# jiangzhengkai/mxdetection

Measured on AMD Instinct MI355X. Metric: images/sec (whole node) Faster R-CNN R50-FPN 3x800x1333, higher is better.
Workload: dtype bf16; 1 GPU; Faster R-CNN ResNet-50-FPN bf16 train step, batch 2/GPU, 3x800x1333 (padded 1344); global_batch=2, parallelism=dp1, frozen=stem+C2, frozen BN folded, optimizer=SGD momentum 0.9 wd 1e-4, launch=hipGraph replay, input=resident, wgrad_side_stream=True, rpn_branch_stream=True, grouped_wgrad=True, filter_prefetch_hints=True, params_trainable=41538304

## Files before the change

include/mxdet.h:

```cpp
#ifndef MXDET_H_
#define MXDET_H_

#include <stddef.h>
#include <stdint.h>

#ifdef __cplusplus
extern "C" {
#endif

#define MXDET_OK 0
#define MXDET_EINVAL (-1)
#define MXDET_ESHAPE (-2)
#define MXDET_EWORKSPACE (-3)
#define MXDET_EHIP (-4)
#define MXDET_ERCCL (-5)

#define MXDET_DTYPE_F32 0
#define MXDET_DTYPE_BF16 1

typedef void* mxdet_stream_t;

const char* mxdet_last_error(void);
const char* mxdet_version(void);

// ... 205 lines not shown
                     const float* bias, const uint16_t* residual, uint16_t* y,
                     mxdet_stream_t stream);
int mxdet_conv2d_fwd_chain(const mxdet_conv_desc_t* d, const uint16_t* x, const uint16_t* w, const float* bias,
                           const uint16_t* w2, const float* bias2, int32_t cout2, int32_t relu2,
                           const uint16_t* residual2, uint16_t* y2, const uint16_t* w3, const float* bias3,
                           int32_t cout3, int32_t relu3, uint16_t* y3, mxdet_stream_t stream);
size_t mxdet_conv2d_fwd_splitk_workspace_bytes(const mxdet_conv_desc_t* d, int32_t ksplit);
int mxdet_conv2d_fwd_splitk(const mxdet_conv_desc_t* d, const uint16_t* x, const uint16_t* w, const float* bias,
                            const uint16_t* residual, uint16_t* y, int32_t ksplit, void* workspace,
                            size_t workspace_bytes, mxdet_stream_t stream);
int mxdet_conv2d_dgrad(const mxdet_conv_desc_t* d, const uint16_t* dy, const uint16_t* wt,
                       const uint16_t* residual, const uint16_t* relu_mask, uint16_t* dx,
                       mxdet_stream_t stream);
size_t mxdet_conv2d_wgrad_workspace_bytes(const mxdet_conv_desc_t* d);
int mxdet_conv2d_wgrad(const mxdet_conv_desc_t* d, const uint16_t* x, const uint16_t* dy, float* dw,
                       float* db, void* workspace, size_t workspace_bytes, mxdet_stream_t stream);
typedef struct {
  mxdet_conv_desc_t desc;
  const void* src;
  const void* filt;
  const float* bias;
  const void* residual;
  const void* relu_mask;
  void* dst;
} mxdet_conv_item_t;
size_t mxdet_conv2d_grouped_table_bytes(int32_t n);
int mxdet_conv2d_grouped_plan(const mxdet_conv_item_t* items, int32_t n, int32_t kind, void* table_host,
                              size_t table_bytes, int32_t* cfg, int32_t* grid);
int mxdet_conv2d_grouped(const void* table_dev, int32_t n, int32_t kind, int32_t cfg, int32_t grid,
                         mxdet_stream_t stream);
typedef struct {
  mxdet_conv_desc_t desc;
  const void* x;
  const void* dy;
  float* dw;
  float* db;
} mxdet_wgrad_item_t;
size_t mxdet_conv2d_wgrad_grouped_table_bytes(int32_t n);
int mxdet_conv2d_wgrad_grouped_plan(const mxdet_wgrad_item_t* items, int32_t n, void* table_host, size_t table_bytes,
                                    size_t* workspace_bytes, int32_t* grid_wgrad, int32_t* grid_big,
                                    int32_t* grid_reduce);
int mxdet_conv2d_wgrad_grouped(const void* table_dev, int32_t n, int32_t grid_wgrad, int32_t grid_big,
                               int32_t grid_reduce, void* workspace, size_t workspace_bytes, size_t workspace_needed,
                               mxdet_stream_t stream);
int mxdet_conv2d_wgrad_grouped_parts(const void* table_dev, int32_t n, int32_t grid_wgrad, int32_t grid_big,
                                     int32_t grid_reduce, int32_t parts, void* workspace, size_t workspace_bytes,
                                     size_t workspace_needed, mxdet_stream_t stream);
int mxdet_filter_transpose(const uint16_t* w, int32_t Cout, int32_t KH, int32_t KW, int32_t Cin,
                           uint16_t* wt, mxdet_stream_t stream);

int mxdet_filter_transpose_batched(const void* descs_dev, int32_t ndesc, int32_t total_tiles,
                                   mxdet_stream_t stream);

typedef struct {
  int32_t N, H, W, C;
  int32_t Ho, Wo;
  int32_t KH, KW;
  int32_t stride, pad;
  int32_t groups;
  int32_t modulated;
  int32_t off_channels;
  int32_t accumulate;
} mxdet_deform_desc_t;
int mxdet_deform_im2col(const mxdet_deform_desc_t* d, const uint16_t* x, const uint16_t* off, uint16_t* col,
                        mxdet_stream_t stream);
int mxdet_deform_col2im_coord(const mxdet_deform_desc_t* d, const uint16_t* x, const uint16_t* off,
                              const uint16_t* dcol, uint16_t* doff, mxdet_stream_t stream);
size_t mxdet_deform_col2im_workspace_bytes(const mxdet_deform_desc_t* d);
int mxdet_deform_col2im(const mxdet_deform_desc_t* d, const uint16_t* off, const uint16_t* dcol, uint16_t* dx,
                        void* workspace, size_t workspace_bytes, mxdet_stream_t stream);

typedef struct {
  int32_t N, HW, C, G;
  float eps;
  int32_t relu;
  int32_t accumulate;
} mxdet_gn_desc_t;
size_t mxdet_group_norm_workspace_bytes(const mxdet_gn_desc_t* d, int32_t backward);
int mxdet_group_norm_fwd(const mxdet_gn_desc_t* d, const uint16_t* x, const float* gamma, const float* beta, uint16_t* y,
                         float* mean, float* rstd, void* workspace, size_t workspace_bytes, mxdet_stream_t stream);
int mxdet_group_norm_bwd(const mxdet_gn_desc_t* d, const uint16_t* x, const uint16_t* dy, const uint16_t* y,
                         const float* mean, const float* rstd, const float* gamma, const float* beta, uint16_t* dx,
                         float* dgamma, float* dbeta, void* workspace, size_t workspace_bytes, mxdet_stream_t stream);

int mxdet_stem_conv7x7(const void* image, int32_t dtype, int32_t N, int32_t H, int32_t W,
                       const uint16_t* w, const float* bias, uint16_t* y, mxdet_stream_t stream);
int mxdet_stem_conv7x7_pool(const void* image, int32_t dtype, int32_t N, int32_t H, int32_t W,
                            const uint16_t* w, const float* bias, uint16_t* y, mxdet_stream_t stream);
int mxdet_maxpool3x3s2(const uint16_t* x, int32_t N, int32_t H, int32_t W, int32_t C, uint16_t* y,
                       mxdet_stream_t stream);
int mxdet_subsample2(const uint16_t* x, int32_t N, int32_t H, int32_t W, int32_t C, uint16_t* y,
                     mxdet_stream_t stream);
int mxdet_subsample2_bwd(const uint16_t* dy, int32_t N, int32_t H, int32_t W, int32_t C,
                         int32_t accumulate, uint16_t* dx, mxdet_stream_t stream);
int mxdet_upsample2_bwd(const uint16_t* dfine, int32_t N, int32_t Hf, int32_t Wf, int32_t C,
                        int32_t accumulate, uint16_t* dcoarse, mxdet_stream_t stream);
size_t mxdet_retina_detect_workspace_bytes(const mxdet_pyramid_t* p, int32_t N, int32_t pre_nms_top_n);
int mxdet_retina_detect(const mxdet_pyramid_t* p, int32_t N, const float* im_info, int32_t pre_nms_top_n,
                        float score_thresh, float nms_thresh, int32_t max_per_image, float* dets, int32_t* num_dets,
                        void* workspace, size_t workspace_bytes, mxdet_stream_t stream);
int mxdet_retina_detect_soft(const mxdet_pyramid_t* p, int32_t N, const float* im_info, int32_t pre_nms_top_n,
                             float score_thresh, float nms_thresh, int32_t max_per_image, float* dets,
                             int32_t* num_dets, void* workspace, size_t workspace_bytes, int32_t method, float sigma,
                             mxdet_stream_t stream);

typedef struct {
// ... 50 lines not shown
```

mxdetection_amd/_lib.py:

```python
import ctypes as C
import os

_HERE = os.path.dirname(os.path.abspath(__file__))
LIB_PATH = os.environ.get("MXDET_LIB") or os.path.join(_HERE, "libmxdet_hip.so")

c_i32, c_i64, c_u32, c_f32, c_sz, c_vp = C.c_int32, C.c_int64, C.c_uint32, C.c_float, C.c_size_t, C.c_void_p


class PyramidT(C.Structure):
    _fields_ = [
        ("num_levels", c_i32), ("A", c_i32),
        ("H", c_i32 * 8), ("W", c_i32 * 8), ("stride", c_i32 * 8),
        ("cls", c_vp * 8), ("reg", c_vp * 8),
        ("cls_sn", c_i64 * 8), ("cls_sy", c_i64 * 8), ("cls_sx", c_i64 * 8), ("cls_sa", c_i64 * 8),
        ("reg_sn", c_i64 * 8), ("reg_sy", c_i64 * 8), ("reg_sx", c_i64 * 8), ("reg_sc", c_i64 * 8),
        ("dtype", c_i32), ("classes", c_i32),
        ("base_anchors", c_vp * 8),
    ]


class FeatPyramidT(C.Structure):
    _fields_ = [
        ("num_levels", c_i32), ("lvl_min", c_i32),
        ("H", c_i32 * 8), ("W", c_i32 * 8),
        ("spatial_scale", c_f32 * 8),
        ("feat", c_vp * 8),
    ]


class ImageDescT(C.Structure):
    _fields_ = [("src", C.c_void_p), ("src_h", C.c_int32), ("src_w", C.c_int32), ("dst_h", C.c_int32),
                ("dst_w", C.c_int32), ("flip", C.c_int32), ("pad_", C.c_int32), ("inv_scale", C.c_double)]


class WgradItemT(C.Structure):
    pass


class ConvItemT(C.Structure):
    pass


class ConvDescT(C.Structure):
    _fields_ = [
        ("N", c_i32), ("H", c_i32), ("W", c_i32), ("Cin", c_i32),
        ("Cout", c_i32), ("KH", c_i32), ("KW", c_i32),
        ("stride", c_i32), ("pad", c_i32),
        ("Ho", c_i32), ("Wo", c_i32),
        ("relu", c_i32), ("res_upsample", c_i32), ("accumulate", c_i32),
        ("prefetch", c_vp), ("prefetch_bytes", c_i64), ("relu_bits", c_vp),
    ]


class DeformDescT(C.Structure):
    _fields_ = [
        ("N", c_i32), ("H", c_i32), ("W", c_i32), ("C", c_i32),
        ("Ho", c_i32), ("Wo", c_i32), ("KH", c_i32), ("KW", c_i32),
        ("stride", c_i32), ("pad", c_i32), ("groups", c_i32), ("modulated", c_i32),
        ("off_channels", c_i32), ("accumulate", c_i32),
    ]


class DpoolDescT(C.Structure):
    _fields_ = [
        ("pyr", FeatPyramidT), ("N", c_i32), ("C", c_i32), ("PH", c_i32), ("PW", c_i32),
        ("sample_per_part", c_i32), ("trans_std", c_f32), ("modulated", c_i32),
        ("trans_stride", c_i32), ("mask_stride", c_i32), ("accumulate", c_i32),
    ]


class GnDescT(C.Structure):
    _fields_ = [("N", c_i32), ("HW", c_i32), ("C", c_i32), ("G", c_i32), ("eps", c_f32), ("relu", c_i32),
                ("accumulate", c_i32)]


WgradItemT._fields_ = [("desc", ConvDescT), ("x", c_vp), ("dy", c_vp), ("dw", c_vp), ("db", c_vp)]
ConvItemT._fields_ = [("desc", ConvDescT), ("src", c_vp), ("filt", c_vp), ("bias", c_vp), ("residual", c_vp),
                      ("relu_mask", c_vp), ("dst", c_vp)]

P = C.POINTER

SIGNATURES = {
    "mxdet_last_error": (C.c_char_p, []),
    "mxdet_version": (C.c_char_p, []),
    "mxdet_box_iou": (c_i32, [c_vp, c_i64, c_vp, c_i64, c_vp, c_vp]),
    "mxdet_generate_anchors": (c_i32, [c_vp, c_i32, c_i32, c_i32, c_i32, c_vp, c_vp]),
    "mxdet_nms_batched_workspace_bytes": (c_sz, [c_i32, c_i32]),
    "mxdet_nms_batched": (c_i32, [c_vp, c_vp, c_vp, c_i32, c_i32, c_f32, c_i32, c_vp, c_vp, c_vp, c_sz, c_vp]),
    "mxdet_soft_nms_batched": (c_i32, [c_vp, c_vp, c_vp, c_i32, c_i32, c_i32, c_f32, c_f32, c_f32, c_i32, c_vp, c_vp, c_vp,
                                       c_vp]),
    "mxdet_pixel_shuffle2_inv_relu": (c_i32, [c_vp, c_vp, c_i64, c_i32, c_i32, c_i32, c_vp, c_vp]),
    "mxdet_mask_paste_workspace_bytes": (c_sz, [c_i64, c_i32]),
    "mxdet_mask_paste": (c_i32, [c_vp, c_vp, c_i64, c_i32, c_i32, c_i32, c_i32, c_f32, c_vp, c_vp, c_sz, c_vp]),
    "mxdet_retina_detect_workspace_bytes": (c_sz, [c_vp, c_i32, c_i32]),
    "mxdet_retina_detect": (c_i32, [c_vp, c_i32, c_vp, c_i32, c_f32, c_f32, c_i32, c_vp, c_vp, c_vp, c_sz, c_vp]),
    "mxdet_retina_detect_soft": (c_i32, [c_vp, c_i32, c_vp, c_i32, c_f32, c_f32, c_i32, c_vp, c_vp, c_vp, c_sz, c_i32, c_f32,
                                         c_vp]),
    "mxdet_debug_preprocess_direct": (c_i32, [c_i32]),
    "mxdet_image_preprocess": (c_i32, [c_vp, c_i32, c_i32, c_i32, c_vp, c_vp, c_i32, c_vp, c_vp]),
    "mxdet_polygon_masks": (c_i32, [c_vp, c_vp, c_vp, c_i32, c_i32, c_i32, c_i32, c_vp, c_vp]),
    "mxdet_detection_postprocess_workspace_bytes": (c_sz, [c_i32, c_i32, c_i32]),
    "mxdet_detection_postprocess": (c_i32, [c_vp, c_vp, c_i32, c_i32, c_i32, c_vp, c_vp, c_vp, c_i32, c_i32, c_i32,
                                            P(c_f32), P(c_f32), c_f32, c_f32, c_i32, c_vp, c_vp, c_vp, c_sz, c_vp]),
    "mxdet_detection_postprocess_soft": (c_i32, [c_vp, c_vp, c_i32, c_i32, c_i32, c_vp, c_vp, c_vp, c_i32, c_i32, c_i32,
                                                 P(c_f32), P(c_f32), c_f32, c_f32, c_i32, c_vp, c_vp, c_vp, c_sz, c_i32,
                                                 c_f32, c_vp]),
    "mxdet_proposal_workspace_bytes": (c_sz, [P(PyramidT), c_i32, c_i32]),
    "mxdet_proposal": (c_i32, [P(PyramidT), c_i32, c_vp, c_i32, c_i32, c_f32, c_f32, c_vp, c_vp, c_vp, c_vp,
                               c_vp, c_sz, c_vp]),
    "mxdet_anchor_target_workspace_bytes": (c_sz, [c_i32, c_i64, c_i32]),
    "mxdet_anchor_target": (c_i32, [c_vp, c_i64, c_vp, c_i32, c_i32, c_vp, c_f32, c_f32, c_f32, c_i32, c_f32,
                                    c_u32, c_u32, c_vp, c_u32, c_vp, c_vp, c_vp, c_vp, c_vp, c_sz, c_vp]),
    "mxdet_atss_assign_workspace_bytes": (c_sz, [c_i32, c_i64, c_i32]),
    "mxdet_atss_assign": (c_i32, [c_vp, c_i64, P(c_i64), c_i32, c_vp, c_i32, c_i32, c_i32, c_vp, c_vp, c_vp, c_vp, c_vp, c_sz,
                                  c_vp]),
    "mxdet_proposal_target": (c_i32, [c_vp, c_vp, c_i32, c_vp, c_i32, c_i32, c_i32, c_f32, c_f32, c_f32, c_f32,
                                      c_i32, c_i32, P(c_f32), P(c_f32), c_u32, c_u32, c_vp, c_u32, c_vp, c_vp, c_vp,
                                      c_vp, c_vp, c_vp, c_vp]),
    "mxdet_fpn_level_map": (c_i32, [c_vp, c_i64, c_i32, c_i32, c_vp, c_vp]),
    "mxdet_roi_align_fwd": (c_i32, [P(FeatPyramidT), c_i32, c_i32, c_vp, c_vp, c_i64, c_i32, c_i32, c_i32, c_vp,
                                    c_vp]),
    "mxdet_roi_align_bwd": (c_i32, [P(FeatPyramidT), c_i32, c_i32, c_vp, c_vp, c_i64, c_i32, c_i32, c_i32, c_vp,
                                    c_vp]),
    "mxdet_roi_align_bwd_gather_workspace_bytes": (c_sz, [P(FeatPyramidT), c_i32, c_i64]),
    "mxdet_roi_align_bwd_gather": (c_i32, [P(FeatPyramidT), c_i32, c_i32, c_vp, c_vp, c_i64, c_i32, c_i32, c_i32, c_vp,
                                           c_i32, c_vp, c_sz, c_vp]),
    "mxdet_roi_align_bwd_gather_prepare": (c_i32, [P(FeatPyramidT), c_i32, c_vp, c_vp, c_i64, c_i32, c_i32, c_i32,
                                                   c_vp, c_sz, c_vp]),
    "mxdet_roi_align_bwd_gather_prepared": (c_i32, [P(FeatPyramidT), c_i32, c_i32, c_vp, c_vp, c_i64, c_i32, c_i32, c_i32,
                                                    c_vp, c_i32, c_vp, c_sz, c_vp]),
    "mxdet_smooth_l1_fwd": (c_i32, [c_vp, c_vp, c_vp, c_i64, c_f32, c_vp, c_vp]),
    "mxdet_smooth_l1_bwd": (c_i32, [c_vp, c_vp, c_vp, c_vp, c_i64, c_f32, c_i32, c_vp, c_vp]),
    "mxdet_loss_workspace_bytes": (c_sz, [c_i64]),
    "mxdet_focal_loss": (c_i32, [c_vp, c_i32, c_vp, c_i64, c_i32, c_f32, c_f32, c_f32, c_vp, c_vp, c_vp, c_sz,
                                 c_vp]),
    "mxdet_anchor_class_labels": (c_i32, [c_vp, c_vp, c_vp, c_i32, c_i64, c_i32, c_vp, c_vp, c_vp]),
    "mxdet_retina_loss_num_partials": (c_i32, [c_i32, c_i32, c_i32, c_i32]),
    "mxdet_retina_loss_level": (c_i32, [c_vp, c_vp, c_i32, c_i32, c_i32, c_i32, c_i32, c_i32, c_i32, c_vp, c_vp, c_i64,
                                        c_i64, c_f32, c_f32, c_f32, c_vp, c_f32, c_vp, c_vp, c_vp, c_vp]),
    "mxdet_rpn_loss_num_partials": (c_i32, [c_i32, c_i32, c_i32]),
    "mxdet_rpn_loss_level": (c_i32, [c_vp, c_i32, c_i32, c_i32, c_i32, c_i32, c_vp, c_vp, c_i64, c_i64, c_f32,
                                     c_f32, c_f32, c_vp, c_vp, c_vp]),
    "mxdet_loss_finalize": (c_i32, [c_vp, c_i32, c_i32, c_vp, c_vp]),
    "mxdet_rcnn_loss": (c_i32, [c_vp, c_vp, c_i32, c_i32, c_i32, c_vp, c_vp, c_vp, c_i64, c_i32, c_i32, c_f32,
                                c_f32, c_f32, c_vp, c_vp, c_vp, c_vp, c_sz, c_vp]),
    "mxdet_box_iou_loss": (c_i32, [c_vp, c_vp, c_vp, c_i32, c_i32, c_vp, c_i64, c_i32, c_f32, c_f32, c_f32, c_f32, c_f32, c_vp,
                                   c_vp, c_vp]),
    "mxdet_rcnn_loss_iou": (c_i32, [c_vp, c_vp, c_i32, c_i32, c_i32, c_vp, c_vp, c_vp, c_vp, c_i32, c_i32, c_i64, c_i32, c_i32,
                                    c_i32, c_f32, c_f32, c_f32, c_f32, c_f32, c_f32, c_f32, c_vp, c_vp, c_vp, c_vp, c_sz,
                                    c_vp]),
    "mxdet_retina_loss_level_iou": (c_i32, [c_vp, c_vp, c_i32, c_i32, c_i32, c_i32, c_i32, c_i32, c_i32, c_vp, c_vp, c_vp, c_vp,
                                            c_i32, c_i64, c_i64, c_f32, c_f32, c_i32, c_f32, c_f32, c_f32, c_f32, c_f32, c_vp,
                                            c_f32, c_vp, c_vp, c_vp, c_vp]),
    "mxdet_mask_target": (c_i32, [c_vp, c_vp, c_vp, c_vp, c_i64, c_i32, c_i32, c_i32, c_i32, c_vp, c_vp, c_vp]),
    "mxdet_pixel_shuffle2": (c_i32, [c_vp, c_i64, c_i32, c_i32, c_i32, c_i32, c_vp, c_vp]),
    "mxdet_mask_loss_workspace_bytes": (c_sz, [c_i64, c_i32]),
    "mxdet_mask_loss": (c_i32, [c_vp, c_vp, c_vp, c_i64, c_i32, c_i32, c_f32, c_vp, c_vp, c_vp, c_sz, c_vp]),
    "mxdet_conv2d_fwd": (c_i32, [P(ConvDescT), c_vp, c_vp, c_vp, c_vp, c_vp, c_vp]),
    "mxdet_conv2d_fwd_chain": (c_i32, [P(ConvDescT), c_vp, c_vp, c_vp, c_vp, c_vp, c_i32, c_i32, c_vp, c_vp, c_vp, c_vp, c_i32,
                                       c_i32, c_vp, c_vp]),
    "mxdet_conv2d_fwd_splitk_workspace_bytes": (c_sz, [P(ConvDescT), c_i32]),
    "mxdet_conv2d_fwd_splitk": (c_i32, [P(ConvDescT), c_vp, c_vp, c_vp, c_vp, c_vp, c_i32, c_vp, c_sz, c_vp]),
    "mxdet_conv2d_dgrad": (c_i32, [P(ConvDescT), c_vp, c_vp, c_vp, c_vp, c_vp, c_vp]),
    "mxdet_conv2d_wgrad_workspace_bytes": (c_sz, [P(ConvDescT)]),
    "mxdet_conv2d_wgrad": (c_i32, [P(ConvDescT), c_vp, c_vp, c_vp, c_vp, c_vp, c_sz, c_vp]),
    "mxdet_conv2d_grouped_table_bytes": (c_sz, [c_i32]),
    "mxdet_conv2d_grouped_plan": (c_i32, [P(ConvItemT), c_i32, c_i32, c_vp, c_sz, P(c_i32), P(c_i32)]),
    "mxdet_conv2d_grouped": (c_i32, [c_vp, c_i32, c_i32, c_i32, c_i32, c_vp]),
    "mxdet_conv2d_wgrad_grouped_table_bytes": (c_sz, [c_i32]),
    "mxdet_conv2d_wgrad_grouped_plan": (c_i32, [P(WgradItemT), c_i32, c_vp, c_sz, P(c_sz), P(c_i32), P(c_i32), P(c_i32)]),
    "mxdet_conv2d_wgrad_grouped": (c_i32, [c_vp, c_i32, c_i32, c_i32, c_i32, c_vp, c_sz, c_sz, c_vp]),
    "mxdet_conv2d_wgrad_grouped_parts": (c_i32, [c_vp, c_i32, c_i32, c_i32, c_i32, c_i32, c_vp, c_sz, c_sz, c_vp]),
    "mxdet_debug_force_conv_cfg": (c_i32, [c_i32]),
    "mxdet_debug_force_wgrad_ksplit": (c_i32, [c_i32]),
    "mxdet_filter_transpose": (c_i32, [c_vp, c_i32, c_i32, c_i32, c_i32, c_vp, c_vp]),
    "mxdet_filter_transpose_batched": (c_i32, [c_vp, c_i32, c_i32, c_vp]),
    "mxdet_deform_im2col": (c_i32, [P(DeformDescT), c_vp, c_vp, c_vp, c_vp]),
    "mxdet_deform_col2im_coord": (c_i32, [P(DeformDescT), c_vp, c_vp, c_vp, c_vp, c_vp]),
    "mxdet_deform_col2im_workspace_bytes": (c_sz, [P(DeformDescT)]),
    "mxdet_deform_col2im": (c_i32, [P(DeformDescT), c_vp, c_vp, c_vp, c_vp, c_sz, c_vp]),
    "mxdet_dpool_fwd": (c_i32, [P(DpoolDescT), c_vp, c_vp, c_i64, c_vp, c_vp, c_vp, c_vp]),
    "mxdet_dpool_bwd_trans": (c_i32, [P(DpoolDescT), c_vp, c_vp, c_i64, c_vp, c_vp, c_vp, c_vp, c_vp, c_vp]),
    "mxdet_dpool_bwd_feat_workspace_bytes": (c_sz, [P(DpoolDescT), c_i64]),
    "mxdet_dpool_bwd_feat": (c_i32, [P(DpoolDescT), c_vp, c_vp, c_i64, c_vp, c_vp, c_vp, c_vp, c_sz, c_vp]),
    "mxdet_group_norm_workspace_bytes": (c_sz, [P(GnDescT), c_i32]),
    "mxdet_group_norm_fwd": (c_i32, [P(GnDescT), c_vp, c_vp, c_vp, c_vp, c_vp, c_vp, c_vp, c_sz, c_vp]),
    "mxdet_group_norm_bwd": (c_i32, [P(GnDescT), c_vp, c_vp, c_vp, c_vp, c_vp, c_vp, c_vp, c_vp, c_vp, c_vp, c_vp, c_sz,
                                     c_vp]),
    "mxdet_debug_group_norm_route": (c_i32, [P(GnDescT)]),
    "mxdet_stem_conv7x7": (c_i32, [c_vp, c_i32, c_i32, c_i32, c_i32, c_vp, c_vp, c_vp, c_vp]),
    "mxdet_stem_conv7x7_pool": (c_i32, [c_vp, c_i32, c_i32, c_i32, c_i32, c_vp, c_vp, c_vp, c_vp]),
    "mxdet_maxpool3x3s2": (c_i32, [c_vp, c_i32, c_i32, c_i32, c_i32, c_vp, c_vp]),
    "mxdet_subsample2": (c_i32, [c_vp, c_i32, c_i32, c_i32, c_i32, c_vp, c_vp]),
    "mxdet_subsample2_bwd": (c_i32, [c_vp, c_i32, c_i32, c_i32, c_i32, c_i32, c_vp, c_vp]),
    "mxdet_upsample2_bwd": (c_i32, [c_vp, c_i32, c_i32, c_i32, c_i32, c_i32, c_vp, c_vp]),
    "mxdet_add_bf16": (c_i32, [c_vp, c_vp, c_i64, c_vp, c_vp]),
    "mxdet_relu_bwd_bf16": (c_i32, [c_vp, c_vp, c_i64, c_vp, c_vp]),
    "mxdet_f32_to_bf16": (c_i32, [c_vp, c_i64, c_vp, c_vp]),
    "mxdet_f32_accum_to_bf16": (c_i32, [c_vp, c_i64, c_i32, c_vp, c_vp]),
    "mxdet_nchw_to_nhwc_bf16": (c_i32, [c_vp, c_i32, c_i32, c_i32, c_i32, c_i32, c_vp, c_vp]),
    "mxdet_nhwc_to_nchw_f32": (c_i32, [c_vp, c_i32, c_i32, c_i32, c_i32, c_vp, c_vp]),
    "mxdet_sgd_momentum_update": (c_i32, [c_vp, c_vp, c_vp, c_vp, c_i64, c_f32, c_f32, c_f32, c_f32, c_vp]),
    "mxdet_sgd_momentum_update_sched": (c_i32, [c_vp, c_vp, c_vp, c_vp, c_i64, c_vp, c_f32, c_f32, c_f32, c_vp]),
    "mxdet_comm_unique_id": (c_i32, [c_vp]),
    "mxdet_comm_create": (c_i32, [c_vp, c_i32, c_i32, P(c_vp)]),
    "mxdet_comm_destroy": (c_i32, [c_vp]),
    "mxdet_allreduce_bucket": (c_i32, [c_vp, c_vp, c_i64, c_vp, P(c_i32)]),
    "mxdet_comm_wait": (c_i32, [c_vp, c_i32, c_vp]),
    "mxdet_comm_broadcast": (c_i32, [c_vp, c_vp, c_sz, c_i32, c_vp]),
    "mxdet_debug_set_tuning": (c_i32, [c_i32, c_i64]),
    "mxdet_debug_get_tuning": (c_i64, [c_i32]),
    "mxdet_debug_route_probe": (c_i32, [c_i32]),
    "mxdet_debug_route_read": (c_i32, [P(c_i32), c_i32]),
}

DEBUG_SYMBOLS = ("mxdet_debug_force_conv_cfg", "mxdet_debug_force_wgrad_ksplit", "mxdet_debug_preprocess_direct",
                 "mxdet_debug_set_tuning", "mxdet_debug_get_tuning", "mxdet_debug_route_probe", "mxdet_debug_route_read",
                 "mxdet_debug_group_norm_route")
TUNING_KEYS = {"T64": 0, "T128": 1, "PAR64": 2, "WG_TARGET": 3, "WG_MINSTEPS": 4, "WG_MAXSTEPS": 5, "T3_ENABLE": 6,
               "T3_TARGET": 7, "T3_MINSTEPS": 8, "T3_NS": 9, "TAIL": 10, "WG_NS": 11, "ROI_TABLE": 12, "ROI_ROWS": 13, "STATIC_TAPS": 14,
               "T128W": 15, "T3_MIX": 16, "SPLITK_TILE": 17, "T3_PER_ITEM": 18}
ROUTE_KINDS = {"CONV": 1, "WGRAD": 2, "CONV_GROUPED": 3, "WGRAD_GROUPED": 4, "RETINA_LOSS": 5, "RETINA_LOSS_IOU": 6}

IOU_LOSS_KINDS = {"iou": 0, "giou": 1, "diou": 2}

_lib = None

# ... 43 lines not shown
```

mxdetection_amd/models/rpn_heads/rpn_head.py:

```python
import os

import torch

from ...core import anchor as A_
from ...core import loss as L_
from ...ops import dense
from ...ops.proposal import PyramidProposal
from ..utils.layers import ConvLayer, cached_buf

HEAD_CPAD = 64


RELU_BITS = os.environ.get("MXDET_TUNE_RELU_BITS", "1") == "1"


class RPNHead:
    def __init__(self, channels, strides, arena, ws, device, gen, ratios=(0.5, 1.0, 2.0), scales=(8,),
                 pre_nms_top_n=2000, post_nms_top_n=2000, nms_thresh=0.7, min_size=0.0, batch_size=256,
                 fg_fraction=0.5, fg_thresh=0.7, bg_thresh=0.3, sigma=3.0, seed=99):
        kw = dict(arena=arena, ws=ws, device=device, gen=gen)
        self.A = len(ratios) * len(scales)
        assert 5 * self.A <= HEAD_CPAD
        self.out = ConvLayer("rpn.out", channels, HEAD_CPAD, 1, init_std=0.01, cout_real=5 * self.A, **kw)
        self.conv = ConvLayer("rpn.conv", channels, channels, 3, init_std=0.01, **kw)
        self.strides = list(strides)
        self.base = [torch.from_numpy(A_.generate_base_anchors(s, ratios, scales)).to(device) for s in strides]
        self.proposal = PyramidProposal(self.base, strides, pre_nms_top_n, post_nms_top_n, nms_thresh, min_size)
        self.batch_size, self.fg_fraction, self.fg_thresh, self.bg_thresh = batch_size, fg_fraction, fg_thresh, bg_thresh
        self.sigma, self.seed, self.device, self.C = sigma, seed, device, channels
        self.bufs = {}
        self.anchors = None
        self.level_shapes = None

    def layers(self):
        return [self.out, self.conv]

    def _buf(self, key, shape, dtype=torch.bfloat16, zero=False):
        return cached_buf(self.bufs, key, shape, dtype, self.device, zero)

    def plan(self, p_shapes, g_max):
        for s in p_shapes:
            self.conv.plan(s)
            self.out.plan(s)
        self.level_shapes = [(s[1], s[2]) for s in p_shapes]
        N = p_shapes[0][0]
        self.anchors = torch.cat([A_.generate_anchors(self.base[l], H, W, self.strides[l])
                                  for l, (H, W) in enumerate(self.level_shapes)])
        self.level_offsets = [0]
        for (H, W) in self.level_shapes:
            self.level_offsets.append(self.level_offsets[-1] + H * W * self.A)
        At = self.anchors.shape[0]
        self.at_ws = A_.AnchorTargetWorkspace(N, At, g_max, self.device)
        self.at_out = (torch.empty((N, At), dtype=torch.int32, device=self.device),
                       torch.empty((N, At), dtype=torch.int32, device=self.device),
                       torch.empty((N, At, 4), dtype=torch.float32, device=self.device),
                       torch.empty((N, At), dtype=torch.float32, device=self.device))
        self.nparts = [L_.rpn_loss_num_partials(N, H, W) for (H, W) in self.level_shapes]
        self.partial = torch.zeros((2 * sum(self.nparts),), dtype=torch.float32, device=self.device)
        self.loss = torch.zeros((2,), dtype=torch.float32, device=self.device)

    def forward(self, P):
        self.P = P
        tb = [self._buf("t%d" % l, p.shape) for l, p in enumerate(P)]
        hb = [self._buf("h%d" % l, p.shape[:3] + (HEAD_CPAD,)) for l, p in enumerate(P)]
        self.tbits = [self._buf("tb%d" % l, p.shape[:3] + (p.shape[3] // 8,), dtype=torch.uint8) if RELU_BITS else None
                      for l, p in enumerate(P)]
        self.conv.forward(P[0], relu=True, out=tb[0], bits_out=self.tbits[0])
        dense.conv2d_group("fwd", [self.conv.fwd_call(P[l], relu=True, out=tb[l], bits_out=self.tbits[l])
                                   for l in range(1, len(P))], self.device)
        self.out.forward(tb[0], out=hb[0])
        dense.conv2d_group("fwd", [self.out.fwd_call(tb[l], out=hb[l]) for l in range(1, len(P))], self.device)
        self.t, self.h = tb, hb
        return self.h

    def get_proposals(self, im_info):
        return self.proposal(self.h, self.h, im_info, layout="nhwc_fused")

    def assign_targets(self, gt_boxes, im_info, step, image_offset, step_dev=None):
        labels, _, targets, _ = A_.assign_anchor(self.anchors, gt_boxes, im_info, self.fg_thresh, self.bg_thresh, 0.0,
                                                 self.batch_size, self.fg_fraction, self.seed, step, image_offset,
                                                 self.at_ws, self.at_out, step_dev)
        self._assigned = (labels, targets)

    def loss_and_grad(self, gt_boxes, im_info, step, image_offset, loss_scale=1.0, step_dev=None, assigned=False):
        if not assigned:
            self.assign_targets(gt_boxes, im_info, step, image_offset, step_dev)
        labels, targets = self._assigned
        N = gt_boxes.shape[0]
        norm = 1.0 / float(N * self.batch_size)
        self.gh = []
        off = 0
        for l, h in enumerate(self.h):
            g = self._buf("gh%d" % l, h.shape)
            L_.rpn_loss_level(h, self.A, labels, targets, self.level_offsets[l], self.sigma, norm, loss_scale, g,
                              self.partial[2 * off:])
            off += self.nparts[l]
            self.gh.append(g)
        L_.loss_finalize(self.partial, off, 2, self.loss)
        return self.loss

    def backward(self, dP, dP_has_grad, flush=True):
        L = len(self.h)
        dt = [self._buf("dt%d" % l, self.t[l].shape) for l in range(L)]
        grouped = self.out.ws.grouping
        for l in range(L):
            self.out.backward_weight(self.t[l], self.gh[l], accumulate=(l > 0) and not grouped)
        self.out.backward_data(self.gh[0], self.t[0].shape, relu_mask=self.t[0], out=dt[0], relu_bits=self.tbits[0])
        dense.conv2d_group("dgrad", [self.out.dgrad_call(self.gh[l], self.t[l].shape, relu_mask=self.t[l], out=dt[l],
                                                         relu_bits=self.tbits[l])
                                     for l in range(1, L)], self.device)
        for l in range(L):
            self.conv.backward_weight(self.P[l], dt[l], accumulate=(l > 0) and not grouped)
        self.conv.backward_data(dt[0], self.P[0].shape, accumulate=dP_has_grad[0], out=dP[0])
        dense.conv2d_group("dgrad", [self.conv.dgrad_call(dt[l], self.P[l].shape, accumulate=dP_has_grad[l], out=dP[l])
                                     for l in range(1, L)], self.device)
        if flush:
            self.out.ws.flush()
```

Before: 446.6 images/sec.

## Add sparse RPN head backward over sampled-anchor cells only

Adds HIP kernels that list the feature cells containing sampled anchors (label >= 0) and compute the RPN head's output-conv dgrad and 3x3-conv dgrad only at those cells and their 3x3 neighbourhoods, zeroing dP elsewhere. An optional mode (env=2) also computes the weight gradients sparsely. The default mode keeps dense wgrad but writes a mostly-zero dt map. The aim is to avoid dense dgrad over every pyramid level, since the loss gradient is nonzero at only a few hundred cells. The cost is extra zero-fill passes, a single-block O(n^2) rank sort, and irregular gather access.

```diff
diff --git a/include/mxdet.h b/include/mxdet.h
--- a/include/mxdet.h
+++ b/include/mxdet.h
@@ -281,6 +281,30 @@
 int mxdet_filter_transpose_batched(const void* descs_dev, int32_t ndesc, int32_t total_tiles,
                                    mxdet_stream_t stream);
 
+#define MXDET_RPN_SPARSE_MAX_LEVELS 8
+#define MXDET_RPN_SPARSE_ZERO 1
+#define MXDET_RPN_SPARSE_DT 2
+#define MXDET_RPN_SPARSE_WGRAD 4
+#define MXDET_RPN_SPARSE_DGRAD 8
+#define MXDET_RPN_SPARSE_DTMAP 16
+typedef struct {
+  int32_t num_levels, N, A, C, Ch, smax;
+  int32_t H[MXDET_RPN_SPARSE_MAX_LEVELS], W[MXDET_RPN_SPARSE_MAX_LEVELS];
+  int32_t accumulate[MXDET_RPN_SPARSE_MAX_LEVELS];
+  const void* P[MXDET_RPN_SPARSE_MAX_LEVELS];
+  const void* t[MXDET_RPN_SPARSE_MAX_LEVELS];
+  const void* tbits[MXDET_RPN_SPARSE_MAX_LEVELS];
+  const void* gh[MXDET_RPN_SPARSE_MAX_LEVELS];
+  void* dP[MXDET_RPN_SPARSE_MAX_LEVELS];
+  void* dt[MXDET_RPN_SPARSE_MAX_LEVELS];
+} mxdet_rpn_sparse_t;
+int mxdet_rpn_sparse_list(const mxdet_rpn_sparse_t* d, const int32_t* labels, int32_t* list, int32_t* state,
+                          int32_t* map, mxdet_stream_t stream);
+int mxdet_rpn_sparse_backward(const mxdet_rpn_sparse_t* d, const int32_t* list, const int32_t* state,
+                              const int32_t* map, const uint16_t* wt_out, const uint16_t* wt_conv, uint16_t* dts,
+                              uint16_t* ghs, float* dw_out, float* db_out, float* dw_conv, float* db_conv,
+                              int32_t parts, mxdet_stream_t stream);
+
 typedef struct {
   int32_t N, H, W, C;
   int32_t Ho, Wo;
diff --git a/mxdetection_amd/_lib.py b/mxdetection_amd/_lib.py
--- a/mxdetection_amd/_lib.py
+++ b/mxdetection_amd/_lib.py
@@ -72,6 +72,12 @@
 class GnDescT(C.Structure):
     _fields_ = [("N", c_i32), ("HW", c_i32), ("C", c_i32), ("G", c_i32), ("eps", c_f32), ("relu", c_i32),
                 ("accumulate", c_i32)]
+
+
+class RpnSparseT(C.Structure):
+    _fields_ = [("num_levels", c_i32), ("N", c_i32), ("A", c_i32), ("C", c_i32), ("Ch", c_i32), ("smax", c_i32),
+                ("H", c_i32 * 8), ("W", c_i32 * 8), ("accumulate", c_i32 * 8),
+                ("P", c_vp * 8), ("t", c_vp * 8), ("tbits", c_vp * 8), ("gh", c_vp * 8), ("dP", c_vp * 8), ("dt", c_vp * 8)]
 
 
 WgradItemT._fields_ = [("desc", ConvDescT), ("x", c_vp), ("dy", c_vp), ("dw", c_vp), ("db", c_vp)]
@@ -173,6 +179,9 @@
     "mxdet_conv2d_wgrad_grouped_parts": (c_i32, [c_vp, c_i32, c_i32, c_i32, c_i32, c_i32, c_vp, c_sz, c_sz, c_vp]),
     "mxdet_debug_force_conv_cfg": (c_i32, [c_i32]),
     "mxdet_debug_force_wgrad_ksplit": (c_i32, [c_i32]),
+    "mxdet_rpn_sparse_list": (c_i32, [P(RpnSparseT), c_vp, c_vp, c_vp, c_vp, c_vp]),
+    "mxdet_rpn_sparse_backward": (c_i32, [P(RpnSparseT), c_vp, c_vp, c_vp, c_vp, c_vp, c_vp, c_vp, c_vp, c_vp, c_vp, c_vp,
+                                          c_i32, c_vp]),
     "mxdet_filter_transpose": (c_i32, [c_vp, c_i32, c_i32, c_i32, c_i32, c_vp, c_vp]),
     "mxdet_filter_transpose_batched": (c_i32, [c_vp, c_i32, c_i32, c_vp]),
     "mxdet_deform_im2col": (c_i32, [P(DeformDescT), c_vp, c_vp, c_vp, c_vp]),
diff --git a/mxdetection_amd/csrc/rpn_sparse.hip b/mxdetection_amd/csrc/rpn_sparse.hip
--- /dev/null
+++ b/mxdetection_amd/csrc/rpn_sparse.hip
@@ -0,0 +1,393 @@
+#include "common.h"
+
+namespace mxdet {
+
+constexpr int kSpLevels = MXDET_RPN_SPARSE_MAX_LEVELS;
+constexpr int kSpMaxSlots = 8192;
+
+struct SpGeo {
+  int L, N, A, C, Ch, smax, CT;
+  int H[kSpLevels], W[kSpLevels], coff[kSpLevels + 1];
+  const uint16_t* P[kSpLevels];
+  const uint16_t* t[kSpLevels];
+  const unsigned char* tbits[kSpLevels];
+  const uint16_t* gh[kSpLevels];
+  uint16_t* dP[kSpLevels];
+  uint16_t* dt[kSpLevels];
+  int acc[kSpLevels];
+  const int* list;
+  const int* state;
+  const int* map;
+  const uint16_t* wt_out;
+  const uint16_t* wt_conv;
+  uint16_t* dts;
+  uint16_t* ghs;
+  float* dw_out;
+  float* db_out;
+  float* dw_conv;
+  float* db_conv;
+};
+
+struct SpCell { int n, l, h, w, pix; };
+
+__device__ __forceinline__ SpCell sp_decode(const SpGeo& g, int cell) {
+  SpCell c;
+  c.n = cell / g.CT;
+  const int gc = cell - c.n * g.CT;
+  int l = 0;
+#pragma unroll
+  for (int i = 1; i < kSpLevels; ++i)
+    if (i < g.L && gc >= g.coff[i]) l = i;
+  c.l = l;
+  const int local = gc - g.coff[l];
+  c.h = local / g.W[l];
+  c.w = local - c.h * g.W[l];
+  c.pix = c.n * g.H[l] * g.W[l] + local;
+  return c;
+}
+
+__device__ __forceinline__ uint16_t sp_bf16(float v) { return (uint16_t)(pack_bf16x2(v, 0.0f) & 0xffffu); }
+
+__global__ void __launch_bounds__(256)
+rpn_sparse_mark_kernel(const int32_t* __restrict__ labels, int cells, int A, int smax, int* __restrict__ list,
+                       int* __restrict__ state, int* __restrict__ map) {
+  const int g = blockIdx.x * 256 + threadIdx.x;
+  if (g >= cells) return;
+  bool act = false;
+  for (int a = 0; a < A; ++a) act = act || labels[(long long)g * A + a] >= 0;
+  map[g] = -1;
+  if (act) {
+    const int pos = atomicAdd(&state[1], 1);
+    if (pos < smax) list[smax + pos] = g;
+  }
+}
+
+__global__ void __launch_bounds__(1024)
+rpn_sparse_sort_kernel(int smax, int* __restrict__ list, int* __restrict__ state, int* __restrict__ map) {
+  __shared__ int keys[kSpMaxSlots];
+  int cnt = state[1];
+  cnt = cnt < smax ? cnt : smax;
+  for (int i = threadIdx.x; i < cnt; i += 1024) keys[i] = list[smax + i];
+  __syncthreads();
+  for (int i = threadIdx.x; i < smax; i += 1024) {
+    if (i < cnt) {
+      const int k = keys[i];
+      int rank = 0;
+      for (int j = 0; j < cnt; ++j) rank += keys[j] < k ? 1 : 0;
+      list[rank] = k;
+      map[k] = rank;
+    } else {
+      list[i] = -1;
+    }
+  }
+  if (threadIdx.x == 0) state[0] = cnt;
+}
+
+__global__ void __launch_bounds__(256) rpn_sparse_zero_kernel(uint4* __restrict__ p, long long n16) {
+  const long long i = (long long)blockIdx.x * 256 + threadIdx.x;
+  if (i < n16) p[i] = make_uint4(0u, 0u, 0u, 0u);
+}
+
+__global__ void __launch_bounds__(64) rpn_sparse_dt_kernel(const SpGeo g) {
+  const int lane = threadIdx.x, frow = lane & 15, fq = lane >> 4;
+  const int S = g.state[0];
+  const int s = blockIdx.x * 16 + frow;
+  const bool ok = s < S;
+  SpCell c = {0, 0, 0, 0, 0};
+  if (ok) c = sp_decode(g, g.list[s]);
+  const bf16x8_t zero = __builtin_bit_cast(bf16x8_t, make_uint4(0u, 0u, 0u, 0u));
+  bf16x8_t a0 = zero, a1 = zero;
+  if (ok) {
+    const uint16_t* row = g.gh[c.l] + (size_t)c.pix * g.Ch;
+    a0 = *(const bf16x8_t*)(row + fq * 8);
+    a1 = *(const bf16x8_t*)(row + 32 + fq * 8);
+  }
+  if (s < g.smax) {
+    *(bf16x8_t*)(g.ghs + (size_t)s * g.Ch + fq * 8) = a0;
+    *(bf16x8_t*)(g.ghs + (size_t)s * g.Ch + 32 + fq * 8) = a1;
+  }
+  for (int j = 0; j < g.C / 16; ++j) {
+    const uint16_t* wr = g.wt_out + (size_t)(j * 16 + frow) * g.Ch;
+    const bf16x8_t b0 = *(const bf16x8_t*)(wr + fq * 8), b1 = *(const bf16x8_t*)(wr + 32 + fq * 8);
+    f32x4_t acc = {0.f, 0.f, 0.f, 0.f};
+    acc = __builtin_amdgcn_mfma_f32_16x16x32_bf16(a0, b0, acc, 0, 0, 0);
+    acc = __builtin_amdgcn_mfma_f32_16x16x32_bf16(a1, b1, acc, 0, 0, 0);
+    const int ci = j * 16 + frow;
+#pragma unroll
+    for (int r = 0; r < 4; ++r) {
+      const int row = fq * 4 + r;
+      const int rok = __shfl((int)ok, row), rl = __shfl(c.l, row), rpix = __shfl(c.pix, row);
+      float v = acc[r] + 0.0f;
+      if (rok) {
+        bool on;
+        const size_t e = (size_t)rpix * g.C + ci;
+        if (g.tbits[rl]) on = (g.tbits[rl][e >> 3] >> (ci & 7)) & 1u;
+        else { const unsigned m = g.t[rl][e]; on = m != 0u && m < 0x8000u; }
+        if (!on) v = 0.0f;
+      }
+      const int srow = blockIdx.x * 16 + row;
+      const uint16_t o = sp_bf16(v);
+      if (srow < g.smax) g.dts[(size_t)srow * g.C + ci] = o;
+      if (rok && g.dt[rl]) g.dt[rl][(size_t)rpix * g.C + ci] = o;
+    }
+  }
+}
+
+__global__ void __launch_bounds__(256) rpn_sparse_wgrad_kernel(const SpGeo g) {
+  constexpr int LD = 68;
+  __shared__ __attribute__((aligned(16))) uint16_t Xs[32 * LD];
+  __shared__ __attribute__((aligned(16))) uint16_t Ys[32 * LD];
+  const int tid = threadIdx.x, lane = tid & 63, frow = lane & 15, fq = lane >> 4;
+  const int wid = __builtin_amdgcn_readfirstlane(tid >> 6);
+  const int ct = g.C / 64;
+  const int nconv = 9 * ct * ct;
+  int b = blockIdx.x;
+  const uint16_t* X;
+  const bool conv = b < nconv;
+  int ldx, x0, y0, dh, dw, ldw;
+  float* out;
+  float* bias = nullptr;
+  if (conv) {
+    const int tap = b / (ct * ct), r = b - tap * ct * ct, cot = r / ct, cit = r - cot * ct;
+    X = g.dts; ldx = g.C; x0 = cot * 64; y0 = cit * 64; dh = tap / 3 - 1; dw = tap % 3 - 1;
+    ldw = 9 * g.C;
+    out = g.dw_conv + (size_t)x0 * ldw + tap * g.C + y0;
+    if (tap == 0 && cit == 0) bias = g.db_conv + x0;
+  } else {
+    b -= nconv;
+    const int cit = b;
+    X = g.ghs; ldx = g.Ch; x0 = 0; y0 = cit * 64; dh = 0; dw = 0;
+    ldw = g.C;
+    out = g.dw_out + y0;
+    if (cit == 0) bias = g.db_out;
+  }
+  const int S = g.state[0];
+  const int lr = tid >> 3, lc = tid & 7;
+  f32x4_t acc[4];
+#pragma unroll
+  for (int j = 0; j < 4; ++j) acc[j] = f32x4_t{0.f, 0.f, 0.f, 0.f};
+  float bsum = 0.0f;
+  for (int k0 = 0; k0 < S; k0 += 32) {
+    const int s = k0 + lr;
+    uint4 xv = make_uint4(0u, 0u, 0u, 0u), yv = xv;
+    if (s < S) {
+      xv = *(const uint4*)(X + (size_t)s * ldx + x0 + lc * 8);
+      const SpCell c = sp_decode(g, g.list[s]);
+      const int hh = c.h + dh, ww = c.w + dw;
+      const uint16_t* y = conv ? g.P[c.l] : g.t[c.l];
+      if (hh >= 0 && hh < g.H[c.l] && ww >= 0 && ww < g.W[c.l])
+        yv = *(const uint4*)(y + ((size_t)(c.n * g.H[c.l] + hh) * g.W[c.l] + ww) * g.C + y0 + lc * 8);
+    }
+    __syncthreads();
+    *(uint2*)(Xs + lr * LD + lc * 8) = make_uint2(xv.x, xv.y);
+    *(uint2*)(Xs + lr * LD + lc * 8 + 4) = make_uint2(xv.z, xv.w);
+    *(uint2*)(Ys + lr * LD + lc * 8) = make_uint2(yv.x, yv.y);
+    *(uint2*)(Ys + lr * LD + lc * 8 + 4) = make_uint2(yv.z, yv.w);
+    __syncthreads();
+    unsigned af[4];
+#pragma unroll
+    for (int e = 0; e < 4; ++e)
+      af[e] = (unsigned)Xs[(fq * 8 + 2 * e) * LD + wid * 16 + frow] |
+              ((unsigned)Xs[(fq * 8 + 2 * e + 1) * LD + wid * 16 + frow] << 16);
+    const bf16x8_t a = __builtin_bit_cast(bf16x8_t, make_uint4(af[0], af[1], af[2], af[3]));
+#pragma unroll
+    for (int j = 0; j < 4; ++j) {
+      unsigned bf[4];
+#pragma unroll
+      for (int e = 0; e < 4; ++e)
+        bf[e] = (unsigned)Ys[(fq * 8 + 2 * e) * LD + j * 16 + frow] |
+                ((unsigned)Ys[(fq * 8 + 2 * e + 1) * LD + j * 16 + frow] << 16);
+      acc[j] = __builtin_amdgcn_mfma_f32_16x16x32_bf16(a, __builtin_bit_cast(bf16x8_t, make_uint4(bf[0], bf[1], bf[2], bf[3])),
+                                                       acc[j], 0, 0, 0);
+    }
+    if (bias != nullptr && tid < 64) {
+      for (int r = 0; r < 32; ++r) bsum += bf16_bits_to_f32(Xs[r * LD + tid]);
+    }
+  }
+#pragma unroll
+  for (int j = 0; j < 4; ++j)
+#pragma unroll
+    for (int r = 0; r < 4; ++r)
+      out[(size_t)(wid * 16 + fq * 4 + r) * ldw + j * 16 + frow] = acc[j][r];
+  if (bias != nullptr && tid < 64) bias[tid] = bsum;
+}
+
+__global__ void __launch_bounds__(256) rpn_sparse_dgrad_kernel(const SpGeo g) {
+  const int lane = threadIdx.x & 63, frow = lane & 15, fq = lane >> 4;
+  const int wid = __builtin_amdgcn_readfirstlane(threadIdx.x >> 6);
+  const int S = g.state[0];
+  const int m = blockIdx.x * 16 + frow;
+  const int tap_m = m / g.smax, s = m - tap_m * g.smax;
+  int src[9];
+#pragma unroll
+  for (int t = 0; t < 9; ++t) src[t] = -1;
+  int dl = 0, dpix = -1;
+  if (tap_m < 9 && s < S) {
+    const int cell = g.list[s];
+    const SpCell c = sp_decode(g, cell);
+    const int H = g.H[c.l], W = g.W[c.l];
+    const int hd = c.h - 1 + tap_m / 3, wd = c.w - 1 + tap_m % 3;
+    if (hd >= 0 && hd < H && wd >= 0 && wd < W) {
+      bool owner = true;
+#pragma unroll
+      for (int t = 0; t < 9; ++t) {
+        const int hs = hd + 1 - t / 3, ws = wd + 1 - t % 3;
+        int sl = -1;
+        if (hs >= 0 && hs < H && ws >= 0 && ws < W) sl = g.map[cell + (hs - c.h) * W + (ws - c.w)];
+        if (t < tap_m && sl >= 0) owner = false;
+        src[t] = sl;
+      }
+      if (owner) { dl = c.l; dpix = (c.n * H + hd) * W + wd; }
+    }
+  }
+  if (dpix < 0) {
+#pragma unroll
+    for (int t = 0; t < 9; ++t) src[t] = -1;
+  }
+  if (__ballot(dpix >= 0) == 0ull) return;
+  const bf16x8_t zero = __builtin_bit_cast(bf16x8_t, make_uint4(0u, 0u, 0u, 0u));
+  const int K9 = 9 * g.C;
+  for (int cit = wid; cit < g.C / 64; cit += 4) {
+    f32x4_t acc[4];
+#pragma unroll
+    for (int j = 0; j < 4; ++j) acc[j] = f32x4_t{0.f, 0.f, 0.f, 0.f};
+    const uint16_t* wbase = g.wt_conv + (size_t)(cit * 64 + frow) * K9 + fq * 8;
+    for (int c0 = 0; c0 < g.C; c0 += 64) {
+#pragma unroll
+      for (int t = 0; t < 9; ++t) {
+        if (__ballot(src[t] >= 0) == 0ull) continue;
+#pragma unroll
+        for (int hf = 0; hf < 2; ++hf) {
+          const int k = c0 + hf * 32;
+          bf16x8_t a = zero;
+          if (src[t] >= 0) a = *(const bf16x8_t*)(g.dts + (size_t)src[t] * g.C + k + fq * 8);
+#pragma unroll
+          for (int j = 0; j < 4; ++j) {
+            const bf16x8_t bw = *(const bf16x8_t*)(wbase + (size_t)j * 16 * K9 + t * g.C + k);
+            acc[j] = __builtin_amdgcn_mfma_f32_16x16x32_bf16(a, bw, acc[j], 0, 0, 0);
+          }
+        }
+      }
+    }
+#pragma unroll
+    for (int r = 0; r < 4; ++r) {
+      const int row = fq * 4 + r;
+      const int rl = __shfl(dl, row), rpix = __shfl(dpix, row);
+      if (rpix < 0) continue;
+      uint16_t* drow = g.dP[rl] + (size_t)rpix * g.C + cit * 64 + frow;
+      const bool accum = g.acc[rl] != 0;
+#pragma unroll
+      for (int j = 0; j < 4; ++j) {
+        float v = acc[j][r] + 0.0f;
+        if (accum) v += bf16_bits_to_f32(drow[j * 16]);
+        drow[j * 16] = sp_bf16(v);
+      }
+    }
+  }
+}
+
+static int sp_zero_levels(const SpGeo& g, uint16_t* const* ptr, const int* skip, hipStream_t s) {
+  for (int l = 0; l < g.L;) {
+    if (skip && skip[l]) { ++l; continue; }
+    MXDET_REQUIRE(ptr[l] != nullptr && ((uintptr_t)ptr[l] & 15) == 0, MXDET_EINVAL, "rpn_sparse_backward: level %d null / unaligned", l);
+    char* p0 = (char*)ptr[l];
+    char* p1 = p0;
+    while (l < g.L && !(skip && skip[l]) && (char*)ptr[l] == p1) {
+      p1 += (size_t)g.N * g.H[l] * g.W[l] * g.C * 2;
+      ++l;
+    }
+    const long long n16 = (long long)(p1 - p0) / 16;
+    hipLaunchKernelGGL(rpn_sparse_zero_kernel, dim3((unsigned)ceil_div<long long>(n16, 256)), dim3(256), 0, s, (uint4*)p0, n16);
+  }
+  return MXDET_OK;
+}
+
+static int sp_fill(SpGeo& g, const mxdet_rpn_sparse_t* d, const char* who) {
+  MXDET_REQUIRE(d != nullptr, MXDET_EINVAL, "%s: null descriptor", who);
+  MXDET_REQUIRE(d->num_levels > 0 && d->num_levels <= kSpLevels && d->N > 0 && d->A > 0, MXDET_ESHAPE,
+                "%s: 1..%d levels, N > 0, A > 0", who, kSpLevels);
+  MXDET_REQUIRE(d->C > 0 && d->C % 64 == 0 && d->Ch == 64, MXDET_ESHAPE, "%s: C %d must be a multiple of 64 and Ch %d must be 64",
+                who, d->C, d->Ch);
+  MXDET_REQUIRE(d->smax > 0 && d->smax <= kSpMaxSlots, MXDET_ESHAPE, "%s: smax %d must be in 1..%d", who, d->smax, kSpMaxSlots);
+  memset(&g, 0, sizeof(g));
+  g.L = d->num_levels; g.N = d->N; g.A = d->A; g.C = d->C; g.Ch = d->Ch; g.smax = d->smax;
+  long long ct = 0;
+  for (int l = 0; l < g.L; ++l) {
+    MXDET_REQUIRE(d->H[l] > 0 && d->W[l] > 0, MXDET_ESHAPE, "%s: level %d is empty", who, l);
+    g.H[l] = d->H[l]; g.W[l] = d->W[l]; g.coff[l] = (int)ct;
+    ct += (long long)d->H[l] * d->W[l];
+    MXDET_REQUIRE((long long)d->N * d->H[l] * d->W[l] * d->C < (1ll << 31), MXDET_ESHAPE, "%s: level %d exceeds 2^31 elements", who, l);
+  }
+  MXDET_REQUIRE((long long)d->N * ct * d->A < (1ll << 31), MXDET_ESHAPE, "%s: more than 2^31 anchors", who);
+  g.coff[g.L] = (int)ct;
+  g.CT = (int)ct;
+  return MXDET_OK;
+}
+
+}
+
+using namespace mxdet;
+
+extern "C" int mxdet_rpn_sparse_list(const mxdet_rpn_sparse_t* d, const int32_t* labels, int32_t* list, int32_t* state,
+                                     int32_t* map, mxdet_stream_t stream) {
+  clear_error();
+  SpGeo g;
+  int rc = sp_fill(g, d, "rpn_sparse_list");
+  if (rc) return rc;
+  MXDET_REQUIRE(labels && list && state && map, MXDET_EINVAL, "rpn_sparse_list: null pointer");
+  hipStream_t s = as_stream(stream);
+  const int cells = g.N * g.CT;
+  if (zero_async(state + 1, sizeof(int32_t), s) != hipSuccess) return check_launch("rpn_sparse_list");
+  hipLaunchKernelGGL(rpn_sparse_mark_kernel, dim3((unsigned)ceil_div(cells, 256)), dim3(256), 0, s, labels, cells, g.A, g.smax,
+                     list, state, map);
+  hipLaunchKernelGGL(rpn_sparse_sort_kernel, dim3(1), dim3(1024), 0, s, g.smax, list, state, map);
+  return check_launch("rpn_sparse_list");
+}
+
+extern "C" int mxdet_rpn_sparse_backward(const mxdet_rpn_sparse_t* d, const int32_t* list, const int32_t* state,
+                                         const int32_t* map, const uint16_t* wt_out, const uint16_t* wt_conv, uint16_t* dts,
+                                         uint16_t* ghs, float* dw_out, float* db_out, float* dw_conv, float* db_conv,
+                                         int32_t parts, mxdet_stream_t stream) {
+  clear_error();
+  SpGeo g;
+  int rc = sp_fill(g, d, "rpn_sparse_backward");
+  if (rc) return rc;
+  MXDET_REQUIRE(list && state && map && dts && ghs, MXDET_EINVAL, "rpn_sparse_backward: null pointer");
+  g.list = list; g.state = state; g.map = map; g.wt_out = wt_out; g.wt_conv = wt_conv; g.dts = dts; g.ghs = ghs;
+  g.dw_out = dw_out; g.db_out = db_out; g.dw_conv = dw_conv; g.db_conv = db_conv;
+  for (int l = 0; l < g.L; ++l) {
+    g.P[l] = (const uint16_t*)d->P[l]; g.t[l] = (const uint16_t*)d->t[l]; g.tbits[l] = (const unsigned char*)d->tbits[l];
+    g.gh[l] = (const uint16_t*)d->gh[l]; g.dP[l] = (uint16_t*)d->dP[l]; g.acc[l] = d->accumulate[l];
+  }
+  hipStream_t s = as_stream(stream);
+  if (parts & MXDET_RPN_SPARSE_ZERO) {
+    rc = sp_zero_levels(g, g.dP, g.acc, s);
+    if (rc) return rc;
+  }
+  if (parts & MXDET_RPN_SPARSE_DTMAP) {
+    MXDET_REQUIRE(parts & MXDET_RPN_SPARSE_DT, MXDET_EINVAL, "rpn_sparse_backward: DTMAP needs DT");
+    for (int l = 0; l < g.L; ++l) g.dt[l] = (uint16_t*)d->dt[l];
+    rc = sp_zero_levels(g, g.dt, nullptr, s);
+    if (rc) return rc;
+  }
+  if (parts & MXDET_RPN_SPARSE_DT) {
+    MXDET_REQUIRE(wt_out, MXDET_EINVAL, "rpn_sparse_backward: null wt_out");
+    for (int l = 0; l < g.L; ++l)
+      MXDET_REQUIRE(g.gh[l] && (g.tbits[l] || g.t[l]), MXDET_EINVAL, "rpn_sparse_backward: level %d: null gh / mask", l);
+    hipLaunchKernelGGL(rpn_sparse_dt_kernel, dim3((unsigned)ceil_div(g.smax, 16)), dim3(64), 0, s, g);
+  }
+  if (parts & MXDET_RPN_SPARSE_WGRAD) {
+    MXDET_REQUIRE(dw_out && db_out && dw_conv && db_conv, MXDET_EINVAL, "rpn_sparse_backward: null weight-gradient pointer");
+    for (int l = 0; l < g.L; ++l)
+      MXDET_REQUIRE(g.P[l] && g.t[l], MXDET_EINVAL, "rpn_sparse_backward: level %d: null P / t", l);
+    const int ct = g.C / 64;
+    hipLaunchKernelGGL(rpn_sparse_wgrad_kernel, dim3((unsigned)(9 * ct * ct + ct)), dim3(256), 0, s, g);
+  }
+  if (parts & MXDET_RPN_SPARSE_DGRAD) {
+    MXDET_REQUIRE(wt_conv, MXDET_EINVAL, "rpn_sparse_backward: null wt_conv");
+    for (int l = 0; l < g.L; ++l)
+      MXDET_REQUIRE(g.dP[l], MXDET_EINVAL, "rpn_sparse_backward: level %d: null dP", l);
+    hipLaunchKernelGGL(rpn_sparse_dgrad_kernel, dim3((unsigned)ceil_div(9 * g.smax, 16)), dim3(256), 0, s, g);
+  }
+  return check_launch("rpn_sparse_backward");
+}
diff --git a/mxdetection_amd/models/rpn_heads/rpn_head.py b/mxdetection_amd/models/rpn_heads/rpn_head.py
--- a/mxdetection_amd/models/rpn_heads/rpn_head.py
+++ b/mxdetection_amd/models/rpn_heads/rpn_head.py
@@ -6,12 +6,15 @@
 from ...core import loss as L_
 from ...ops import dense
 from ...ops.proposal import PyramidProposal
+from ...ops import rpn_sparse as RS
+from ...ops.rpn_sparse import MAX_SLOTS, RPNSparse
 from ..utils.layers import ConvLayer, cached_buf
 
 HEAD_CPAD = 64
 
 
 RELU_BITS = os.environ.get("MXDET_TUNE_RELU_BITS", "1") == "1"
+RPN_SPARSE = int(os.environ.get("MXDET_TUNE_RPN_SPARSE", "1"))
 
 
 class RPNHead:
@@ -58,6 +61,18 @@
         self.nparts = [L_.rpn_loss_num_partials(N, H, W) for (H, W) in self.level_shapes]
         self.partial = torch.zeros((2 * sum(self.nparts),), dtype=torch.float32, device=self.device)
         self.loss = torch.zeros((2,), dtype=torch.float32, device=self.device)
+        smax = N * self.batch_size
+        self.sparse = (RPNSparse(self.level_shapes, N, self.A, self.C, HEAD_CPAD, smax, self.device)
+                       if RPN_SPARSE and 0 < smax <= MAX_SLOTS else None)
+        self.sparse_wgrad = int(RPN_SPARSE) == 2
+        self.dt_map = None
+        if self.sparse is not None and not self.sparse_wgrad:
+            sizes = [s[0] * s[1] * s[2] * s[3] for s in p_shapes]
+            flat = self._buf("dt_map", (sum(sizes),))
+            self.dt_map, off = [], 0
+            for s, n in zip(p_shapes, sizes):
+                self.dt_map.append(flat[off:off + n].view(tuple(s)))
+                off += n
 
     def forward(self, P):
         self.P = P
@@ -81,6 +96,8 @@
                                                  self.batch_size, self.fg_fraction, self.seed, step, image_offset,
                                                  self.at_ws, self.at_out, step_dev)
         self._assigned = (labels, targets)
+        if self.sparse is not None:
+            self.sparse.build_list(labels)
 
     def loss_and_grad(self, gt_boxes, im_info, step, image_offset, loss_scale=1.0, step_dev=None, assigned=False):
         if not assigned:
@@ -100,6 +117,8 @@
         return self.loss
 
     def backward(self, dP, dP_has_grad, flush=True):
+        if self.sparse is not None:
+            return self._backward_sparse(dP, dP_has_grad, flush)
         L = len(self.h)
         dt = [self._buf("dt%d" % l, self.t[l].shape) for l in range(L)]
         grouped = self.out.ws.grouping
@@ -116,3 +135,20 @@
                                      for l in range(1, L)], self.device)
         if flush:
             self.out.ws.flush()
+
+    def _backward_sparse(self, dP, dP_has_grad, flush=True):
+        g = self.out.arena
+        grads = (g.view(self.out.wi, "g"), g.view(self.out.bi, "g"), g.view(self.conv.wi, "g"), g.view(self.conv.bi, "g"))
+        if self.sparse_wgrad:
+            self.sparse.backward(self.P, self.t, self.tbits, self.gh, dP, dP_has_grad, self.out.wt, self.conv.wt, *grads)
+            return
+        L = len(self.h)
+        grouped = self.out.ws.grouping
+        for l in range(L):
+            self.out.backward_weight(self.t[l], self.gh[l], accumulate=(l > 0) and not grouped)
+        self.sparse.backward(self.P, self.t, self.tbits, self.gh, dP, dP_has_grad, self.out.wt, self.conv.wt, *grads,
+                             parts=RS.ZERO | RS.DT | RS.DTMAP | RS.DGRAD, dt=self.dt_map)
+        for l in range(L):
+            self.conv.backward_weight(self.P[l], self.dt_map[l], accumulate=(l > 0) and not grouped)
+        if flush:
+            self.out.ws.flush()
diff --git a/mxdetection_amd/ops/rpn_sparse.py b/mxdetection_amd/ops/rpn_sparse.py
--- /dev/null
+++ b/mxdetection_amd/ops/rpn_sparse.py
@@ -0,0 +1,53 @@
+import ctypes as C
+
+import torch
+
+from .. import _lib
+from .._lib import RpnSparseT, check, ptr, stream_ptr
+
+ZERO, DT, WGRAD, DGRAD, DTMAP = 1, 2, 4, 8, 16
+ALL = ZERO | DT | WGRAD | DGRAD
+MAX_SLOTS = 8192
+
+
+class RPNSparse:
+
+    def __init__(self, level_shapes, N, A, C_, Ch, smax, device):
+        self.level_shapes, self.N, self.A, self.C, self.Ch, self.smax = list(level_shapes), N, A, C_, Ch, smax
+        self.CT = sum(h * w for h, w in level_shapes)
+        i32 = dict(dtype=torch.int32, device=device)
+        self.list = torch.full((2 * smax,), -1, **i32)
+        self.state = torch.zeros((2,), **i32)
+        self.map = torch.full((N * self.CT,), -1, **i32)
+        self.dts = torch.zeros((smax, C_), dtype=torch.bfloat16, device=device)
+        self.ghs = torch.zeros((smax, Ch), dtype=torch.bfloat16, device=device)
+        self._descs = {}
+
+    def _desc(self, P=None, t=None, tbits=None, gh=None, dP=None, accumulate=None, dt=None):
+        L = len(self.level_shapes)
+        ops = (P, t, tbits, gh, dP, dt)
+        key = tuple(None if o is None else tuple(0 if x is None else x.data_ptr() for x in o) for o in ops)
+        key += (None if accumulate is None else tuple(bool(a) for a in accumulate),)
+        d = self._descs.get(key)
+        if d is None:
+            d = RpnSparseT()
+            d.num_levels, d.N, d.A, d.C, d.Ch, d.smax = L, self.N, self.A, self.C, self.Ch, self.smax
+            for l, (h, w) in enumerate(self.level_shapes):
+                d.H[l], d.W[l] = h, w
+                d.accumulate[l] = int(bool(accumulate[l])) if accumulate is not None else 0
+                for name, o in zip(("P", "t", "tbits", "gh", "dP", "dt"), ops):
+                    if o is not None and o[l] is not None:
+                        getattr(d, name)[l] = o[l].data_ptr()
+            self._descs[key] = d
+        return d
+
+    def build_list(self, labels):
+        assert labels.dtype == torch.int32 and labels.numel() == self.N * self.CT * self.A and labels.is_contiguous()
+        check(_lib.load().mxdet_rpn_sparse_list(C.byref(self._desc()), ptr(labels), ptr(self.list), ptr(self.state),
+                                                ptr(self.map), stream_ptr()), "rpn_sparse_list")
+
+    def backward(self, P, t, tbits, gh, dP, accumulate, wt_out, wt_conv, dw_out, db_out, dw_conv, db_conv, parts=ALL, dt=None):
+        d = self._desc(P, t, tbits, gh, dP, accumulate, dt)
+        check(_lib.load().mxdet_rpn_sparse_backward(C.byref(d), ptr(self.list), ptr(self.state), ptr(self.map), ptr(wt_out),
+                                                    ptr(wt_conv), ptr(self.dts), ptr(self.ghs), ptr(dw_out), ptr(db_out),
+                                                    ptr(dw_conv), ptr(db_conv), parts, stream_ptr()), "rpn_sparse_backward")
```

Result: faster. 451.7 images/sec (median of 6 runs) (+1.2%).
